# Jiang-Muyun/PointNet12

Measured on AMD Instinct MI355X. Metric: points/sec fwd+bwd, PointNet2 SemSeg B=16x4096 pts, higher is better.
Workload: dtype f32 (wide-layer products: exact bf16x3 operand splits, 6 bf16 MFMAs per fp32 product, fp32 accumulate)

## Files before the change

### pointnet12_amd/csrc/mlp_res.hip

```cpp
#include "mlp_loaders.h"
#include "split_bf16.h"
#include <algorithm>

int pn2_wide_fwd(const float *X, int ldx, const float *in_affine, const float *W, int ldw, const float *bias, float *Y, int ldy,
                 int64_t P, int K, int N, double *stats, LazyBn lz, hipStream_t s, int64_t *rows_done, int Kpool,
                 const float *pool_gamma, float *pool_ws);

namespace {

constexpr int RES_BM = 64;

struct ResPlan {
    signed char dx_rb[8], dx_cj[8];
    signed char dw_cj[8], dw_q0[8], dw_q1[8];
};

inline bool make_res_plan(int CI_T, ResPlan *out) {
    ResPlan p;
    int load[8], next_q[4] = {0, 0, 0, 0};
    for (int w = 0; w < 8; ++w) { p.dx_rb[w] = p.dx_cj[w] = -1; p.dw_cj[w] = 0; p.dw_q0[w] = p.dw_q1[w] = 0; load[w] = 0; }
    if (CI_T < 1 || CI_T > 4) return false;
    for (int i = 0; i < 2 * CI_T; ++i) { p.dx_rb[i] = (signed char)(i & 1); p.dx_cj[i] = (signed char)(i >> 1); load[i] = 2; }
    const int target = CI_T > 2 ? CI_T : 2;
    for (int pass = 0; pass < 2; ++pass)
// ... 686 lines not shown
                        const float4 a0 = xr[0], a1 = xr[1], a2 = xr[2];
                        g0[0] = __builtin_fmaf(dz, a0.x, g0[0]); g0[FUSE0 ? 1 : 0] = __builtin_fmaf(dz, a0.y, g0[FUSE0 ? 1 : 0]);
                        g0[FUSE0 ? 2 : 0] = __builtin_fmaf(dz, a0.z, g0[FUSE0 ? 2 : 0]); g0[FUSE0 ? 3 : 0] = __builtin_fmaf(dz, a0.w, g0[FUSE0 ? 3 : 0]);
                        g0[FUSE0 ? 4 : 0] = __builtin_fmaf(dz, a1.x, g0[FUSE0 ? 4 : 0]); g0[FUSE0 ? 5 : 0] = __builtin_fmaf(dz, a1.y, g0[FUSE0 ? 5 : 0]);
                        g0[FUSE0 ? 6 : 0] = __builtin_fmaf(dz, a1.z, g0[FUSE0 ? 6 : 0]); g0[FUSE0 ? 7 : 0] = __builtin_fmaf(dz, a1.w, g0[FUSE0 ? 7 : 0]);
                        g0[FUSE0 ? 8 : 0] = __builtin_fmaf(dz, a2.x, g0[FUSE0 ? 8 : 0]); g0[FUSE0 ? 9 : 0] = __builtin_fmaf(dz, a2.y, g0[FUSE0 ? 9 : 0]);
                        g0[FUSE0 ? 10 : 0] = __builtin_fmaf(dz, a2.z, g0[FUSE0 ? 10 : 0]); g0[FUSE0 ? 11 : 0] = __builtin_fmaf(dz, a2.w, g0[FUSE0 ? 11 : 0]);
                    } else {
#if defined(PN2_EXP_NOSTORE)
                        if (dz == 1.2345e-33f) xb[offx] = dz;
#elif defined(PN2_EXP_PLAINSTORE)
                        xb[offx] = dz;
#else
                        PN2_STREAM_STORE(dz, xb + offx);
#endif
                    }
                    offx += ((r & 3) == 3 ? 5u : 1u) * (unsigned)ldxo;
                }
                if (MASKED) { st0 += (double)s0; st1 += (double)s1; }
                RSTAMP(4)
            }
            chunk += G;
            buf ^= 1;
        };
        while (chunk < chunks) {
            iter(D2 ? raw1 : raw0);
            if (chunk >= chunks) break;
            iter(raw0);
        }
        RSTAMP_FLUSH(wave)
        RABS(wave, 2)
        if (!DXW) {
#pragma unroll
            for (int j = 0; j < TW; ++j) {
                const int e = (wave - CI_T) + j * NDW;
                if (e < NTILE) {
                    const int mb = e / CI_T, nb = e - mb * CI_T;
#pragma unroll
                    for (int r = 0; r < 16; ++r)
                        atomicAdd(dW + (int64_t)(mb * 32 + acc_row(r, lh)) * lddw + nb * 32 + l31, accw[DXW ? 0 : j][r]);
                }
            }
        } else if (MASKED && red_p != nullptr) {
            st0 += __shfl_xor(st0, 32, 64);
            st1 += __shfl_xor(st1, 32, 64);
            if (lh == 0) {
                double *rep = red_p + (size_t)(blockIdx.x % PN2_STAT_REPLICAS) * 2 * Ci;
                atomicAdd(rep + ecol, st0);
                atomicAdd(rep + Ci + ecol, st1);
            }
        }
        if (DXW && FUSE0) {
#pragma unroll
            for (int j = 0; j < (DXW && FUSE0 ? 12 : 1); ++j) g0[j] += __shfl_xor(g0[j], 32, 64);
            if (lh == 0) {
                float *pr = part0 + ((size_t)(blockIdx.x % PN2_CF_REPL) * Ci + ecol) * 16;
#pragma unroll
                for (int j = 0; j < (DXW && FUSE0 ? 12 : 1); ++j) atomicAdd(pr + j, g0[j]);
            }
        }
    };
    if (has_dx) run(pn2_true{}); else run(pn2_false{});
    RABS(wave, 3)
}

template <int CO_T, int CI_T, bool POOLED, bool MASKED, bool FUSE0 = false>
int launch_split_bwd_res(ResDy dy, const float *Yp, int ldp, const float *aff_p, const float *W, int ldw, int64_t tiles, float *dX, int ldxo,
                         double *red_p, float *dW, int lddw, hipStream_t s, const float *X0 = nullptr, int ld0 = 0, float *part0 = nullptr) {
    constexpr int Co = 32 * CO_T, Ci = 32 * CI_T;
    constexpr size_t lds = 2 * 6 * (size_t)(32 * 256) + sizeof(float) * (2 * 32 * (Ci + 4) + 8 * Co + 6 * Ci + (FUSE0 ? 2 * 32 * 12 : 0)) +
                           (CO_T == 4 && CI_T < 4 ? (size_t)CI_T * (Co / 16) * 1024 : 0);
    static_assert(lds <= 160 * 1024, "LDS");
    if ((reinterpret_cast<uintptr_t>(dy.Y) & 15) != 0 || (reinterpret_cast<uintptr_t>(Yp) & 15) != 0) return PN2_EUNSUPPORTED;
    auto kern = split_bwd_res_kernel<CO_T, CI_T, POOLED, MASKED, FUSE0>;
    static Pn2PerDevice raised;
    if (pn2_raise_dynamic_lds(reinterpret_cast<const void *>(kern), raised) != PN2_OK) return PN2_ELAUNCH;
    const int64_t chunks = tiles * (RES_BM / 32), cap = pn2_num_cus();
    PN2_NOTE_KERNEL(kern);
    hipLaunchKernelGGL(kern, dim3((unsigned)(chunks < cap ? chunks : cap)), dim3(512), lds, s, dy, Yp, ldp, aff_p, W, ldw, chunks, dX, ldxo,
                       red_p, dW, lddw, X0, ld0, part0);
    return pn2_launch_status();
}

template <int CO_T, int CI_T>
__global__ __launch_bounds__(512, 1) void split_bwd_cf_kernel(const float *dZp, const int32_t *arg, int ldo, int kshift, const float *W2 ,
                                                              const float *Yp, int ldp, const float *aff_p, int64_t chunks, float *dX, int ldxo, double *red_p,
                                                              float *slab) {
    constexpr int Co = 32 * CO_T, Ci = 32 * CI_T, BP = 32, QD = Co / 4, QP = Ci / 4, LDP = Ci + 4;
    constexpr int PANEL = BP * 256, BUF = 6 * PANEL;
    constexpr int KBX = Co / 16, KBM = Ci / 16, KBT = KBX + KBM;
    constexpr int NS = 8 - CI_T - 1, NTS = 64 * NS;
    constexpr int NGT = CI_T * (CI_T + 1) / 2, LDT = Co + Ci + 4;
    static_assert(NS >= CO_T, "one staging wave per D column");
    constexpr int RPP = NTS / QD, IT_D = (BP + RPP - 1) / RPP, IT_P = (BP * QP + NTS - 1) / NTS;
    static_assert(NTS % QD == 0, "one channel quad of D per staging thread");
    unsigned char *lds_b = reinterpret_cast<unsigned char *>(res_lds);
    float *Yps = res_lds + (2 * BUF) / 4;
    float *xtab = Yps + 2 * BP * LDP;
    const int t = threadIdx.x, lane = t & 63, wave = __builtin_amdgcn_readfirstlane(t >> 6), l31 = lane & 31, lh = lane >> 5;
    const int G = gridDim.x;
    RABS(wave, 0)
    for (int i = t; i < 3 * Ci; i += 512) { const float v = aff_p[i]; xtab[i] = v; xtab[3 * Ci + i] = i < Ci ? v : -v; }

    const bool has_dx = wave < CI_T, is_gram = wave == CI_T;
    const int ecol = (has_dx ? wave : 0) * 32 + l31;
    const int ts = wave <= CI_T ? 0 : t - 64 * (CI_T + 1);
    struct Raw { float4 z; int4 a; float4 p[IT_P]; };
    Raw raw;
    auto p_item = [&](int i, int &row, int &q) { const int idx = (NTS * (i + 1) > BP * QP) ? min(ts + NTS * i, BP * QP - 1) : ts + NTS * i; row = idx / QP; q = idx - row * QP; };
    auto fetch = [&](int64_t chunk) {
        const unsigned m0 = (unsigned)(chunk < chunks ? chunk : chunks - 1) * BP;
        const unsigned o = (m0 >> kshift) * (unsigned)ldo + 4u * (unsigned)(ts % QD);
        raw.z = ld4(dZp + o);
        raw.a = ld4i(arg + o);
#pragma unroll
        for (int i = 0; i < IT_P; ++i) {
            int row, q;
            p_item(i, row, q);
            raw.p[i] = ld4(Yp + ((m0 + (unsigned)row) * (unsigned)ldp + 4u * (unsigned)q));
        }
    };
    auto store_split = [&](unsigned char *img, int row, int q, const float4 v) {
        unsigned h0, m0, l0, h1, m1, l1;
        split2(v.x, v.y, h0, m0, l0);
        split2(v.z, v.w, h1, m1, l1);
        const unsigned o = tr_img_off(row, q >> 1) + 8u * (unsigned)(q & 1);
        *reinterpret_cast<uint2 *>(img + o) = make_uint2(h0, h1);
        *reinterpret_cast<uint2 *>(img + o + PANEL) = make_uint2(m0, m1);
        *reinterpret_cast<uint2 *>(img + o + 2 * PANEL) = make_uint2(l0, l1);
    };
    auto stage = [&](int64_t chunk, int buf) {
        unsigned char *ia = lds_b + buf * BUF, *ib = ia + 3 * PANEL;
        float *yp = Yps + buf * (BP * LDP);
        const unsigned m0 = (unsigned)(chunk < chunks ? chunk : chunks - 1) * BP;
        const int kbase = (int)(m0 & ((1u << kshift) - 1u));
        const int par = (int)(chunk & 1);
        const float *xt = xtab + par * (3 * Ci);
        const float lim = par ? -INFINITY : INFINITY;
        {
            unsigned h0, m0_, l0, h1, m1, l1;
            split2(raw.z.x, raw.z.y, h0, m0_, l0);
            split2(raw.z.z, raw.z.w, h1, m1, l1);
            const unsigned sm2 = par ? 0x80008000u : 0u;
            h0 ^= sm2; m0_ ^= sm2; l0 ^= sm2; h1 ^= sm2; m1 ^= sm2; l1 ^= sm2;
            const int q = ts % QD, r0 = ts / QD;
            const int4 a = raw.a;
#pragma unroll
            for (int i = 0; i < IT_D; ++i) {
                const int row = (RPP * (i + 1) > BP) ? min(r0 + RPP * i, BP - 1) : r0 + RPP * i;
                const int k = kbase + row;
                const unsigned k0 = (a.x == k ? 0x0000ffffu : 0u) | (a.y == k ? 0xffff0000u : 0u);
                const unsigned k1 = (a.z == k ? 0x0000ffffu : 0u) | (a.w == k ? 0xffff0000u : 0u);
                const unsigned o = tr_img_off(row, q >> 1) + 8u * (unsigned)(q & 1);
                *reinterpret_cast<uint2 *>(ia + o) = make_uint2(h0 & k0, h1 & k1);
                *reinterpret_cast<uint2 *>(ia + o + PANEL) = make_uint2(m0_ & k0, m1 & k1);
                *reinterpret_cast<uint2 *>(ia + o + 2 * PANEL) = make_uint2(l0 & k0, l1 & k1);
            }
        }
#pragma unroll
        for (int i = 0; i < IT_P; ++i) {
            int row, q;
            p_item(i, row, q);
            float4 x = raw.p[i];
            *reinterpret_cast<float4 *>(&yp[row * LDP + 4 * q]) = x;
            const float4 mu = *reinterpret_cast<const float4 *>(&xt[4 * q]), sc = *reinterpret_cast<const float4 *>(&xt[Ci + 4 * q]);
            const float4 be = *reinterpret_cast<const float4 *>(&xt[2 * Ci + 4 * q]);
            x.x = __builtin_amdgcn_fmed3f(bn_act(x.x, mu.x, sc.x, be.x), 0.f, lim); x.y = __builtin_amdgcn_fmed3f(bn_act(x.y, mu.y, sc.y, be.y), 0.f, lim);
            x.z = __builtin_amdgcn_fmed3f(bn_act(x.z, mu.z, sc.z, be.z), 0.f, lim); x.w = __builtin_amdgcn_fmed3f(bn_act(x.w, mu.w, sc.w, be.w), 0.f, lim);
            store_split(ib, row, q, x);
        }
    };
    auto raw_landed = [&]() {
        asm volatile("" : "+v"(raw.z.x), "+v"(raw.z.y), "+v"(raw.z.z), "+v"(raw.z.w));
        asm volatile("" : "+v"(raw.a.x), "+v"(raw.a.y), "+v"(raw.a.z), "+v"(raw.a.w));
#pragma unroll
        for (int i = 0; i < IT_P; ++i) asm volatile("" : "+v"(raw.p[i].x), "+v"(raw.p[i].y), "+v"(raw.p[i].z), "+v"(raw.p[i].w));
    };
    const int g16 = lane >> 4, j16 = lane & 15, tq = j16 >> 2, tp = j16 & 3;
    auto frag_t = [&](const unsigned char *img, int cblk, int pb) {
        const int c0 = (cblk * 32 + 16 * (g16 & 1)) >> 3;
        SplitFrag f;
#pragma unroll
        for (int r2 = 0; r2 < 2; ++r2) {
            const int row = 16 * pb + 8 * (g16 >> 1) + 4 * r2 + tq;
            const unsigned o = tr_img_off(row, c0 + (tp >> 1)) + 8u * (unsigned)(tp & 1);
            const pn2_s16x4 v = __builtin_amdgcn_ds_read_tr16_b64_v4i16(
                reinterpret_cast<__attribute__((address_space(3))) pn2_s16x4 *>((__attribute__((address_space(3))) unsigned char *)(img) + o));
            const uint2 u = __builtin_bit_cast(uint2, v);
            f.u[2 * r2] = u.x; f.u[2 * r2 + 1] = u.y;
        }
        return f;
    };

    if (has_dx) {
        SplitFrag wh[KBT], wm[KBT], wl[KBM];
        uint4 *wl_lds = reinterpret_cast<uint4 *>(xtab + 6 * Ci) + (size_t)wave * KBX * 64 + lane;
        {
            float v[KBT][8];
#pragma unroll
            for (int kb = 0; kb < KBT; ++kb)
#pragma unroll
                for (int e = 0; e < 8; ++e) v[kb][e] = W2[(16 * kb + 8 * lh + e) * Ci + ecol];
#pragma unroll
            for (int kb = 0; kb < KBT; ++kb) {
                SplitFrag lo;
#pragma unroll
                for (int e = 0; e < 4; ++e) split2(v[kb][2 * e], v[kb][2 * e + 1], wh[kb].u[e], wm[kb].u[e], lo.u[e]);
                if (kb < KBX) wl_lds[kb * 64] = lo.q; else wl[kb < KBX ? 0 : kb - KBX] = lo;
            }
        }
        Affine a(aff_p, Ci);
        const float emu = a.mean[ecol], esc = a.scale[ecol], ebe = a.beta[ecol], eis = a.invstd[ecol];
        const float eh = W2[(Co + Ci) * Ci + ecol];
        double st0 = 0.0, st1 = 0.0, st2 = 0.0;
        int64_t chunk = blockIdx.x;
        int buf = 0;
        __syncthreads();
        RABS(wave, 1)
        RSTAMP_DECL
        while (chunk < chunks) {
            __syncthreads();
            RSTAMP(2)
            const unsigned char *ia = lds_b + buf * BUF, *ib = ia + 3 * PANEL;
            f32x16 acc, acc2;
#pragma unroll
            for (int r = 0; r < 16; ++r) { acc[r] = 0.f; acc2[r] = 0.f; }
#ifndef PN2_X_CF_NODXM
#pragma unroll
            for (int kb = 0; kb < KBT; ++kb) {
                const unsigned char *img = kb < KBX ? ia : ib;
                const unsigned o = tr_img_off(l31, 2 * (kb < KBX ? kb : kb - KBX) + lh);
                SplitFrag ah, am, al, wlo;
                ah.q = *reinterpret_cast<const uint4 *>(img + o);
                am.q = *reinterpret_cast<const uint4 *>(img + o + PANEL);
                al.q = *reinterpret_cast<const uint4 *>(img + o + 2 * PANEL);
                if (kb < KBX) wlo.q = wl_lds[kb * 64]; else wlo = wl[kb < KBX ? 0 : kb - KBX];
                acc = __builtin_amdgcn_mfma_f32_32x32x16_bf16(al.v, wh[kb].v, acc, 0, 0, 0);
                acc2 = __builtin_amdgcn_mfma_f32_32x32x16_bf16(ah.v, wlo.v, acc2, 0, 0, 0);
                acc = __builtin_amdgcn_mfma_f32_32x32x16_bf16(am.v, wm[kb].v, acc, 0, 0, 0);
                acc2 = __builtin_amdgcn_mfma_f32_32x32x16_bf16(am.v, wh[kb].v, acc2, 0, 0, 0);
                acc = __builtin_amdgcn_mfma_f32_32x32x16_bf16(ah.v, wm[kb].v, acc, 0, 0, 0);
                acc2 = __builtin_amdgcn_mfma_f32_32x32x16_bf16(ah.v, wh[kb].v, acc2, 0, 0, 0);
            }
#endif
#ifdef PN2_STAMP
            { float a0_ = acc[0] + acc2[0]; asm volatile("" : "+v"(a0_)); }
#endif
            RSTAMP(3)
#ifdef PN2_X_CF_NOEPI
            if (acc[0] == 1.2345e-33f) dX[0] = acc2[1];
            chunk += G; buf ^= 1;
            continue;
#endif
            const float *yq = Yps + buf * (BP * LDP) + (4 * lh) * LDP + ecol;
            float yv[16];
#pragma unroll
            for (int r = 0; r < 16; ++r) yv[r] = yq[((r & 3) + 8 * (r >> 2)) * LDP];
// ... 27 lines not shown
        if (lh == 0) {
            if (red_p != nullptr) {
                double *rep = red_p + (size_t)(blockIdx.x % PN2_STAT_REPLICAS) * 2 * Ci;
                atomicAdd(rep + ecol, st0);
                atomicAdd(rep + Ci + ecol, st1);
            }
            slab[(size_t)blockIdx.x * (Ci * LDT) + (size_t)ecol * LDT + Co + Ci] = (float)st2;
        }
    } else {
        constexpr int PA[6] = {2, 0, 1, 1, 0, 0}, PB[6] = {0, 2, 1, 0, 1, 0};
        auto mm2 = [&](f32x16 &c0, const SplitFrag (&a0)[3], const SplitFrag (&b0)[3], f32x16 &c1, const SplitFrag (&a1)[3], const SplitFrag (&b1)[3]) {
#pragma unroll
            for (int q = 0; q < 6; ++q) {
                c0 = __builtin_amdgcn_mfma_f32_32x32x16_bf16(a0[PA[q]].v, b0[PB[q]].v, c0, 0, 0, 0);
                c1 = __builtin_amdgcn_mfma_f32_32x32x16_bf16(a1[PA[q]].v, b1[PB[q]].v, c1, 0, 0, 0);
            }
        };
        auto mm1 = [&](f32x16 &c0, const SplitFrag (&a0)[3], const SplitFrag (&b0)[3]) {
#pragma unroll
            for (int q = 0; q < 6; ++q) c0 = __builtin_amdgcn_mfma_f32_32x32x16_bf16(a0[PA[q]].v, b0[PB[q]].v, c0, 0, 0, 0);
        };
        auto frag3 = [&](const unsigned char *img, int blk, int pb, SplitFrag (&f)[3]) {
            f[0] = frag_t(img, blk, pb); f[1] = frag_t(img + PANEL, blk, pb); f[2] = frag_t(img + 2 * PANEL, blk, pb);
        };
        float *sl = slab + (size_t)blockIdx.x * (Ci * LDT);
        if (is_gram) {
            f32x16 accg[NGT];
#pragma unroll
            for (int j = 0; j < NGT; ++j)
#pragma unroll
                for (int r = 0; r < 16; ++r) accg[j][r] = 0.f;
            int64_t chunk = blockIdx.x;
            int buf = 0;
            __syncthreads();
            RABS(wave, 1)
            RSTAMP_DECL
            while (chunk < chunks) {
                __syncthreads();
                RSTAMP(2)
#ifndef PN2_X_CF_NOT
                const unsigned char *ib = lds_b + buf * BUF + 3 * PANEL;
#pragma unroll
                for (int pb = 0; pb < BP / 16; ++pb) {
                    SplitFrag fx[CI_T][3];
#pragma unroll
                    for (int i = 0; i < CI_T; ++i) frag3(ib, i, pb, fx[i]);
                    if constexpr (CI_T == 1) {
                        mm1(accg[0], fx[0], fx[0]);
                    } else if constexpr (CI_T == 2) {
                        mm2(accg[0], fx[0], fx[0], accg[1], fx[0], fx[1]);
                        mm1(accg[2], fx[1], fx[1]);
                    } else {
                        static_assert(CI_T <= 3, "Gram tiles");
                        mm2(accg[0], fx[0], fx[0], accg[1], fx[0], fx[1]);
                        mm2(accg[2], fx[1], fx[1], accg[3], fx[0], fx[2]);
                        mm2(accg[4], fx[1], fx[2], accg[5], fx[2], fx[2]);
                    }
                }
#endif
                RSTAMP(3)
                chunk += G;
                buf ^= 1;
            }
            RSTAMP_FLUSH(wave)
            RABS(wave, 2)
#pragma unroll
            for (int j = 0; j < CI_T; ++j)
#pragma unroll
                for (int i = 0; i <= j; ++i) {
                    const f32x16 &acc = accg[j * (j + 1) / 2 + i];
#pragma unroll
                    for (int r = 0; r < 16; ++r) sl[(i * 32 + acc_row(r, lh)) * LDT + Co + j * 32 + l31] = acc[r];
                    if (i != j) {
#pragma unroll
                        for (int r = 0; r < 16; ++r) sl[(j * 32 + l31) * LDT + Co + i * 32 + acc_row(r, lh)] = acc[r];
                    }
                }
        } else {
            f32x16 accw[CI_T];
#pragma unroll
            for (int j = 0; j < CI_T; ++j)
#pragma unroll
                for (int r = 0; r < 16; ++r) accw[j][r] = 0.f;
            const int nb = wave - CI_T - 1 < CO_T ? wave - CI_T - 1 : -1;
            int64_t chunk = blockIdx.x;
            fetch(chunk);
            __syncthreads();
            stage(chunk, 0);
            fetch(chunk + G);
            raw_landed();
            int buf = 0;
            RABS(wave, 1)
            RSTAMP_DECL
            while (chunk < chunks) {
                __syncthreads();
                RSTAMP(2)
#ifndef PN2_X_CF_NOSTAGE
                stage(chunk + G, buf ^ 1);
#endif
                RSTAMP(0)
#ifndef PN2_X_CF_NOFETCH
                fetch(chunk + 2 * (int64_t)G);
#endif
                __builtin_amdgcn_sched_barrier(0);
                RSTAMP(1)
#ifndef PN2_X_CF_NOT
                if (nb >= 0) {
                    const unsigned char *ia = lds_b + buf * BUF, *ib = ia + 3 * PANEL;
#pragma unroll
                    for (int pb = 0; pb < BP / 16; ++pb) {
                        SplitFrag fb[3], fa0[3], fa1[3];
                        frag3(ia, nb, pb, fb);
                        frag3(ib, 0, pb, fa0);
                        if constexpr (CI_T >= 2) {
                            frag3(ib, 1, pb, fa1);
                            mm2(accw[0], fa0, fb, accw[CI_T >= 2 ? 1 : 0], fa1, fb);
                            if constexpr (CI_T == 3) {
                                frag3(ib, 2, pb, fa0);
                                mm1(accw[CI_T == 3 ? 2 : 0], fa0, fb);
                            }
                        } else {
                            mm1(accw[0], fa0, fb);
                        }
                    }
                }
#endif
                RSTAMP(3)
                chunk += G;
                buf ^= 1;
            }
            RSTAMP_FLUSH(wave)
            RABS(wave, 2)
            if (nb >= 0) {
#pragma unroll
                for (int i = 0; i < CI_T; ++i)
#pragma unroll
                    for (int r = 0; r < 16; ++r) sl[(i * 32 + acc_row(r, lh)) * LDT + nb * 32 + l31] = accw[i][r];
            }
        }
    }
    RABS(wave, 3)
}

__global__ __launch_bounds__(128) void cf_prep_kernel(LazyCoef lc, const float *coef, int ldc, const float *__restrict__ W, int ldw,
                                                      const float *__restrict__ bias, int Co, int Ci, float *__restrict__ W2) {
    __shared__ double fac[256];
    lazy_coef_prologue(lc);
    const float *c0 = coef, *q1 = coef + ldc, *q0 = coef + 2 * ldc, *mean = coef + 3 * ldc;
    const int r = blockIdx.x;
    if (r < Co) {
        for (int i = threadIdx.x; i < Ci; i += 128) W2[r * Ci + i] = c0[r] * W[(int64_t)r * ldw + i];
        return;
    }
    const int j = r - Co;
    for (int c = threadIdx.x; c < Co; c += 128)
        fac[c] = j == Ci ? ((double)q1[c] * ((double)bias[c] - (double)mean[c]) + (double)q0[c]) : (double)W[(int64_t)c * ldw + j] * (double)q1[c];
    __syncthreads();
    for (int i = threadIdx.x; i < Ci; i += 128) {
        double s0 = 0.0, s1 = 0.0, s2 = 0.0, s3 = 0.0;
#pragma unroll 4
        for (int c = 0; c < Co; c += 4) {
            s0 += fac[c] * (double)W[(int64_t)c * ldw + i];
            s1 += fac[c + 1] * (double)W[(int64_t)(c + 1) * ldw + i];
            s2 += fac[c + 2] * (double)W[(int64_t)(c + 2) * ldw + i];
            s3 += fac[c + 3] * (double)W[(int64_t)(c + 3) * ldw + i];
        }
        W2[r * Ci + i] = (float)((s0 + s1) + (s2 + s3));
    }
}

__global__ __launch_bounds__(256) void cf_finish_kernel(const float *__restrict__ slab, int nslab, int Co, int Ci, const float *coef, int ldc,
                                                        const float *__restrict__ W, int ldw, const float *__restrict__ bias,
                                                        float *__restrict__ dW, int lddw) {
    extern __shared__ double cf_row[];
    const int i = blockIdx.x, LDT = Co + Ci + 4, NQ = LDT / 4;
    const int q = threadIdx.x & 63, sg = threadIdx.x >> 6;
    double a0 = 0.0, a1 = 0.0, a2 = 0.0, a3 = 0.0;
    if (q < NQ) {
        const float *p = slab + (size_t)i * LDT + 4 * q;
        const size_t ss = (size_t)Ci * LDT;
        int w = sg;
        for (; w + 28 < nslab; w += 32) {
            float4 v[8];
#pragma unroll
            for (int e = 0; e < 8; ++e) v[e] = ld4(p + (size_t)(w + 4 * e) * ss);
#pragma unroll
            for (int e = 0; e < 8; ++e) { a0 += (double)v[e].x; a1 += (double)v[e].y; a2 += (double)v[e].z; a3 += (double)v[e].w; }
        }
        for (; w < nslab; w += 4) {
            const float4 v = ld4(p + (size_t)w * ss);
            a0 += (double)v.x; a1 += (double)v.y; a2 += (double)v.z; a3 += (double)v.w;
        }
        double *d = cf_row + sg * LDT + 4 * q;
        d[0] = a0; d[1] = a1; d[2] = a2; d[3] = a3;
    }
    __syncthreads();
    for (int n = threadIdx.x; n < LDT; n += 256) cf_row[n] = (cf_row[n] + cf_row[LDT + n]) + (cf_row[2 * LDT + n] + cf_row[3 * LDT + n]);
    __syncthreads();
    const float *c0 = coef, *q1 = coef + ldc, *q0 = coef + 2 * ldc, *mean = coef + 3 * ldc;
    const double sx = cf_row[Co + Ci];
    for (int c = threadIdx.x; c < Co; c += 256) {
        double dot = 0.0;
        for (int j = 0; j < Ci; ++j) dot += (double)W[(int64_t)c * ldw + j] * cf_row[Co + j];
        const double g = (double)c0[c] * cf_row[c] + (double)q1[c] * (dot + ((double)bias[c] - (double)mean[c]) * sx) + (double)q0[c] * sx;
        dW[(int64_t)c * lddw + i] += (float)g;
    }
}

template <int CO_T, int CI_T>
int launch_split_bwd_cf(const float *dZp, const int32_t *arg, int ldo, int kshift, const float *coef, LazyCoef lc, const float *W, int ldw,
                        const float *bias, const float *Yp, int ldp, const float *aff_p, int64_t P, float *dX, int ldxo, double *red_p,
                        float *dW, int lddw, float *scratch, hipStream_t s) {
    constexpr int Co = 32 * CO_T, Ci = 32 * CI_T, LDT = Co + Ci + 4;
    constexpr size_t lds = 2 * 6 * (size_t)(32 * 256) + sizeof(float) * (2 * 32 * (Ci + 4) + 6 * Ci) + (size_t)CI_T * (Co / 16) * 1024;
    static_assert(lds <= 160 * 1024, "LDS");
    auto kern = split_bwd_cf_kernel<CO_T, CI_T>;
    static Pn2PerDevice raised;
    if (pn2_raise_dynamic_lds(reinterpret_cast<const void *>(kern), raised) != PN2_OK) return PN2_ELAUNCH;
    float *W2 = scratch, *slab = scratch + (((Co + Ci + 1) * Ci + 63) & ~63);
    const int64_t chunks = P / 32, cap = pn2_num_cus() < 256 ? pn2_num_cus() : 256;
    const int grid = (int)(chunks < cap ? chunks : cap);
    hipLaunchKernelGGL(cf_prep_kernel, dim3(Co + Ci + 1), dim3(128), 0, s, lc, coef, (Co + 3) & ~3, W, ldw, bias, Co, Ci, W2);
    PN2_NOTE_KERNEL(kern);
    hipLaunchKernelGGL(kern, dim3((unsigned)grid), dim3(512), lds, s, dZp, arg, ldo, kshift, W2, Yp, ldp, aff_p, chunks, dX, ldxo, red_p, slab);
    hipLaunchKernelGGL(cf_finish_kernel, dim3(Ci), dim3(256), sizeof(double) * 4 * LDT, s, slab, grid, Co, Ci, coef, (Co + 3) & ~3, W, ldw, bias,
                       dW, lddw);
    return pn2_launch_status();
}

#define PN2_RES_CASE(CO, CI, POOL, MASKED)                                                                                \
    if (Co == CO && Ci == CI)                                                                                              \
        return launch_bwd_res<CO / 32, CI / 32, POOL, MASKED>(dy, Yp, ldp, aff_p, W, ldw, tiles, dX, ldxo, red_p, dW, lddw, s);

int dispatch_bwd_res(int Kpool, bool masked, int Co, int Ci, ResDy dy, const float *Yp, int ldp, const float *aff_p, const float *W,
                     int ldw, int64_t tiles, float *dX, int ldxo, double *red_p, float *dW, int lddw, hipStream_t s) {
    if (pn2_opt(PN2_OPT_SPLIT) && pn2_opt(PN2_OPT_SPLIT_RES)) {
#define PN2_SPLIT_RES_CASE(CO, CI, POOLED, MASKED)                                                                        \
        if (Co == CO && Ci == CI) {                                                                                        \
            const int rc = launch_split_bwd_res<CO / 32, CI / 32, POOLED, MASKED>(dy, Yp, ldp, aff_p, W, ldw, tiles, dX, ldxo, red_p, dW, lddw, s); \
            if (rc != PN2_EUNSUPPORTED) return rc;                                                                         \
        }
        const bool all = pn2_opt(PN2_OPT_SPLIT_RES) >= 2;
        if (Kpool == 0 && masked) {
            if (all) { PN2_SPLIT_RES_CASE(32, 32, false, true) }
            PN2_SPLIT_RES_CASE(64, 64, false, true) PN2_SPLIT_RES_CASE(96, 64, false, true)
            if (tiles >= pn2_opt(PN2_OPT_SPLIT_RES_MIN_TILES_128)) { PN2_SPLIT_RES_CASE(128, 128, false, true) }
        } else if (Kpool == 0) {
            if (tiles >= pn2_opt(PN2_OPT_SPLIT_RES_MIN_TILES_128)) { PN2_SPLIT_RES_CASE(128, 128, false, false) }
        } else if (masked && Kpool % 32 == 0) {
            if (all) { PN2_SPLIT_RES_CASE(64, 32, true, true) }
            PN2_SPLIT_RES_CASE(128, 64, true, true) PN2_SPLIT_RES_CASE(128, 96, true, true)
        }
#undef PN2_SPLIT_RES_CASE
    }
    if (Kpool == 0 && masked) {
        PN2_RES_CASE(32, 32, 0, true) PN2_RES_CASE(64, 64, 0, true) PN2_RES_CASE(96, 64, 0, true)
        if (tiles >= 4096) { PN2_RES_CASE(128, 128, 0, true) }
    } else if (Kpool == 0) {
        if (tiles >= 4096) { PN2_RES_CASE(128, 128, 0, false) }
    } else if (masked && Kpool % 64 == 0) {
        PN2_RES_CASE(128, 64, 1, true) PN2_RES_CASE(128, 96, 1, true)
    } else if (masked && Kpool == 32) {
        PN2_RES_CASE(64, 32, 2, true) PN2_RES_CASE(128, 64, 2, true)
    }
    return PN2_EUNSUPPORTED;
}

struct ResPool {
    float2 *rec;
    const float *gamma;
    int ldp, U;
    LazyBn lz;
};

template <int K_T, int N_T, bool ACT, int POOL>
__global__ __launch_bounds__(512, 2) void fwd_res_kernel(const float *__restrict__ X, int ldx, const float *aff ,
                                                         const float *__restrict__ W, int ldw, const float *__restrict__ bias,
                                                         float *__restrict__ Y, int ldy, int64_t slabs, double *__restrict__ stats,
                                                         ResPool pool) {
    constexpr int K = 32 * K_T, N = 32 * N_T, LDA = K + 4, QK = K / 4, IT = 32 * QK / 64;
    const int NW = blockDim.x >> 6;
    float *Ws = res_lds;
    float *atab = Ws + N * LDA;
    const int t = threadIdx.x, lane = t & 63, wave = __builtin_amdgcn_readfirstlane(t >> 6), l31 = lane & 31, lh = lane >> 5;
    float *Ab = atab + 3 * K + wave * (32 * LDA);
    RABS(wave, 0)

    lazy_bn_prologue(pool.lz);
    for (int i = t; i < N * QK; i += blockDim.x) {
        const int n = i / QK, q = i - n * QK;
        const float *src = W + (int64_t)n * ldw + 4 * q;
        float4 v;
        if ((ldw & 3) == 0 && (reinterpret_cast<uintptr_t>(W) & 15) == 0) v = ld4(src);
        else v = make_float4(src[0], src[1], src[2], src[3]);
        *reinterpret_cast<float4 *>(&Ws[n * LDA + 4 * q]) = v;
    }
    if (ACT)
        for (int i = t; i < 3 * K; i += blockDim.x) atab[i] = aff[i];
    float bj[N_T];
// ... 326 lines not shown

extern "C" int pn2_bn_pool_select(const float *pool_ws, const float *affine, int64_t G, int C, float *out, int ldo, int32_t *arg,
                                  const pn2_bn_lazy *lazy, pn2_stream_t stream) {
    PN2_CHECK_ARG(lazy_bn_ok(lazy, affine, C));
    PN2_CHECK_ARG(pool_ws && affine && out && arg && G > 0 && C > 0 && C % 32 == 0 && ldo >= C && ldo % 4 == 0 &&
                  (reinterpret_cast<uintptr_t>(pool_ws) & 15) == 0 && (reinterpret_cast<uintptr_t>(out) & 15) == 0);
    const int64_t n = G * (C >> 2);
    int64_t blocks = pn2_cdiv(n, 256);
    const int64_t cap = (int64_t)pn2_num_cus() * 8;
    if (blocks > cap) blocks = cap;
    hipLaunchKernelGGL(bn_pool_select_kernel, dim3((unsigned)blocks), dim3(256), 0, pn2_s(stream),
                       reinterpret_cast<const float2 *>(pool_ws), C, affine, C, G, C, out, ldo, arg, make_lazy_bn(lazy));
    return pn2_launch_status();
}

extern "C" int pn2_conv1x1_bwd(const float *dZ, int ldz, const float *dZp, int ldo, const int32_t *arg, int Kpool, const float *Y,
                               int ldy, const float *coef, const float *W, int ldw, const float *prev_Y, int ld_prev,
                               const float *prev_affine, float *dXout, int ldxo, double *prev_red, float *dW, int lddw,
                               int64_t P, int C_out, int C_in, const pn2_bn_coef_lazy *coef_lazy, pn2_stream_t stream) {
    PN2_CHECK_ARG(Y && coef && W && prev_Y && dXout && dW && P > 0 && P < (1LL << 31) && res_shape_ok(C_out, C_in));
    PN2_CHECK_ARG(lazy_coef_ok(coef_lazy, coef, C_out));
    PN2_CHECK_ARG(dZ != nullptr || (dZp && arg && Kpool > 0));
    PN2_CHECK_ARG(ldw >= C_in && lddw >= C_in && ldy % 4 == 0 && ldy >= C_out && ld_prev % 4 == 0 && ld_prev >= C_in && ldxo >= C_in);
    PN2_CHECK_ARG(prev_affine != nullptr || prev_red == nullptr);
    hipStream_t s = pn2_s(stream);
    const int kshift = dZ ? 0 : pow2_shift(Kpool);
    PN2_CHECK_ARG(dZ ? (ldz == ldy) : (kshift >= 0 && ldo % 4 == 0 && ldo >= C_out && prev_affine != nullptr && P % Kpool == 0));
    int64_t tiles = P / RES_BM, P_full = tiles * RES_BM;
    int rc = PN2_OK;
    const int64_t ld_max = std::max(std::max((int64_t)ldy, (int64_t)ld_prev), std::max((int64_t)ldxo, dZ ? (int64_t)ldz : (int64_t)ldo));
    if (P * ld_max >= (1LL << 32)) { tiles = 0; P_full = 0; }
    if (tiles > 0) {
        ResDy dy{dZ, dZp, arg, ldo, kshift, Y, ldy, coef, make_lazy_coef(coef_lazy)};
        rc = dispatch_bwd_res(dZ ? 0 : Kpool, prev_affine != nullptr, C_out, C_in, dy, prev_Y, ld_prev, prev_affine, W, ldw, tiles, dXout, ldxo,
                              prev_red, dW, lddw, s);
        if (rc == PN2_EUNSUPPORTED) { rc = PN2_OK; tiles = 0; P_full = 0; }
        else coef_lazy = nullptr;
    }
    if (rc != PN2_OK || P_full == P) return rc;
    const int64_t tail = P - P_full;
    const int64_t g_off = dZ ? 0 : (P_full / Kpool) * ldo;
    const float *dZt = dZ ? dZ + P_full * ldz : nullptr;
    const float *dZpt = dZ ? nullptr : dZp + g_off;
    const int32_t *argt = dZ ? nullptr : arg + g_off;
    rc = pn2_conv1x1_dgrad(dZt, ldz, dZpt, ldo, argt, Kpool, Y + P_full * ldy, ldy, coef, W, ldw, prev_affine ? prev_Y + P_full * ld_prev : nullptr,
                           ld_prev, prev_affine, dXout + P_full * ldxo, ldxo, prev_red, tail, C_out, C_in, coef_lazy, stream);
    if (rc != PN2_OK) return rc;
    return pn2_conv1x1_wgrad(dZt, ldz, dZpt, ldo, argt, Kpool, Y + P_full * ldy, ldy, coef, prev_Y + P_full * ld_prev, ld_prev, prev_affine,
                             dW, lddw, nullptr, tail, C_out, C_in, nullptr, stream);
}

static bool cf_shape(int C_out, int C_in) { return C_out == 128 && (C_in == 96 || C_in == 64); }

extern "C" int pn2_conv1x1_bwd_cf_supported(int64_t P, int C_out, int C_in, int Kpool) {
    if (!(pn2_opt(PN2_OPT_SPLIT) && pn2_opt(PN2_OPT_SPLIT_RES) && pn2_opt(PN2_OPT_POOL_CF))) return 0;
    if (!pn2_res_supported(P, C_out, C_in) || !cf_shape(C_out, C_in)) return 0;
    if (C_in == 64 && pn2_opt(PN2_OPT_POOL_CF) < 2) return 0;
    if (Kpool < 32 || (Kpool & (Kpool - 1)) != 0 || P % Kpool != 0) return 0;
    if (P * (int64_t)std::max(C_out, C_in) >= (1LL << 32)) return 0;
    return 1;
}

extern "C" int64_t pn2_conv1x1_bwd_cf_scratch_bytes(int C_out, int C_in) {
    if (!cf_shape(C_out, C_in)) return 0;
    const int64_t w2 = (((int64_t)(C_out + C_in + 1) * C_in + 63) & ~63LL);
    return 4 * (w2 + 256LL * C_in * (C_out + C_in + 4));
}

extern "C" int pn2_conv1x1_bwd_cf(const float *dZp, int ldo, const int32_t *arg, int Kpool, const float *coef, const float *W, int ldw,
                                  const float *bias, const float *prev_Y, int ld_prev, const float *prev_affine, float *dXout, int ldxo,
                                  double *prev_red, float *dW, int lddw, int64_t P, int C_out, int C_in, const pn2_bn_coef_lazy *coef_lazy,
                                  float *scratch, pn2_stream_t stream) {
    PN2_CHECK_ARG(dZp && arg && coef && W && bias && prev_Y && prev_affine && dXout && dW && scratch && P > 0 && P < (1LL << 31));
    PN2_CHECK_ARG(lazy_coef_ok(coef_lazy, coef, C_out));
    PN2_CHECK_ARG(ldw >= C_in && lddw >= C_in && ld_prev % 4 == 0 && ld_prev >= C_in && ldxo >= C_in && ldo % 4 == 0 && ldo >= C_out);
    PN2_CHECK_ARG((reinterpret_cast<uintptr_t>(scratch) & 255) == 0 && (reinterpret_cast<uintptr_t>(prev_Y) & 15) == 0 &&
                  (reinterpret_cast<uintptr_t>(dZp) & 15) == 0 && (reinterpret_cast<uintptr_t>(arg) & 15) == 0);
    if (!pn2_conv1x1_bwd_cf_supported(P, C_out, C_in, Kpool)) return PN2_EUNSUPPORTED;
    const int64_t ld_max = std::max(std::max((int64_t)ld_prev, (int64_t)ldxo), (int64_t)ldo);
    if (P * ld_max >= (1LL << 32)) return PN2_EUNSUPPORTED;
    const int kshift = pow2_shift(Kpool);
    const LazyCoef lc = make_lazy_coef(coef_lazy);
    hipStream_t s = pn2_s(stream);
    if (C_in == 96) return launch_split_bwd_cf<4, 3>(dZp, arg, ldo, kshift, coef, lc, W, ldw, bias, prev_Y, ld_prev, prev_affine, P, dXout, ldxo, prev_red, dW, lddw, scratch, s);
    return launch_split_bwd_cf<4, 2>(dZp, arg, ldo, kshift, coef, lc, W, ldw, bias, prev_Y, ld_prev, prev_affine, P, dXout, ldxo, prev_red, dW, lddw, scratch, s);
}

extern "C" int pn2_conv1x1_bwd_first_supported(int64_t P, int C_out, int C_in, int N0) {
    if (!(pn2_opt(PN2_OPT_SPLIT) && pn2_opt(PN2_OPT_SPLIT_RES) && pn2_opt(PN2_OPT_FUSE_FIRST))) return 0;
    if (!pn2_res_supported(P, C_out, C_in) || P % 64 != 0 || N0 < 1 || N0 > 12) return 0;
    if (P * (int64_t)std::max(C_out, C_in) >= (1LL << 32)) return 0;
    return (C_out == 96 && C_in == 64) || (C_out == 64 && C_in == 64);
}

extern "C" int pn2_conv1x1_bwd_first(const float *dZ, int ldz, const float *Y, int ldy, const float *coef, const float *W, int ldw,
                                     const float *prev_Y, int ld_prev, const float *prev_affine, double *prev_red, float *dW, int lddw,
                                     const float *X0, int ld0, int N0, void *cf_scratch, int64_t P, int C_out, int C_in,
                                     const pn2_bn_coef_lazy *coef_lazy, pn2_stream_t stream) {
    PN2_CHECK_ARG(dZ && Y && coef && W && prev_Y && prev_affine && prev_red && dW && X0 && cf_scratch && P > 0 && P < (1LL << 31));
    PN2_CHECK_ARG(lazy_coef_ok(coef_lazy, coef, C_out));
    PN2_CHECK_ARG(ldz == ldy && ldw >= C_in && lddw >= C_in && ldy % 4 == 0 && ldy >= C_out && ld_prev % 4 == 0 && ld_prev >= C_in);
    PN2_CHECK_ARG(ld0 % 4 == 0 && ld0 >= 12 && (reinterpret_cast<uintptr_t>(X0) & 15) == 0 && (reinterpret_cast<uintptr_t>(cf_scratch) & 15) == 0);
    if (!pn2_conv1x1_bwd_first_supported(P, C_out, C_in, N0)) return PN2_EUNSUPPORTED;
    if (P * (int64_t)std::max((int64_t)ldy, std::max((int64_t)ld_prev, (int64_t)ld0)) >= (1LL << 32)) return PN2_EUNSUPPORTED;
    float *part0 = reinterpret_cast<float *>(reinterpret_cast<double *>(cf_scratch) + PN2_CF_REPL * 256);
    ResDy dy{dZ, nullptr, nullptr, 0, 0, Y, ldy, coef, make_lazy_coef(coef_lazy)};
    const int64_t tiles = P / RES_BM;
    hipStream_t s = pn2_s(stream);
    if (C_out == 96) return launch_split_bwd_res<3, 2, false, true, true>(dy, prev_Y, ld_prev, prev_affine, W, ldw, tiles, nullptr, 0, prev_red, dW, lddw, s, X0, ld0, part0);
    return launch_split_bwd_res<2, 2, false, true, true>(dy, prev_Y, ld_prev, prev_affine, W, ldw, tiles, nullptr, 0, prev_red, dW, lddw, s, X0, ld0, part0);
}
```

### pointnet12_amd/csrc/pn2_common.h

```cpp
#pragma once
#include <hip/hip_runtime.h>
#include <stdint.h>
#include <mutex>
#include <set>
#include <utility>
#include "../../include/pn2.h"

#define PN2_WAVE 64
#define PN2_CF_REPL 8

#ifdef PN2_PLAIN_STORES
#define PN2_STREAM_STORE(value, ptr) (*(ptr) = (value))
#else
#define PN2_STREAM_STORE(value, ptr) __builtin_nontemporal_store((value), (ptr))
#endif

#define PN2_CHECK_ARG(cond) \
    do {                    \
        if (!(cond)) return PN2_EINVAL; \
    } while (0)

static inline int pn2_launch_status() { return hipGetLastError() == hipSuccess ? PN2_OK : PN2_ELAUNCH; }

static inline hipStream_t pn2_s(pn2_stream_t s) { return reinterpret_cast<hipStream_t>(s); }

static inline int64_t pn2_cdiv(int64_t a, int64_t b) { return (a + b - 1) / b; }

#define PN2_OPTION_LIST(X) \
    X(FPS_ROWS_MIN_PPT, 24)  \
    X(FPS_ROWMAP, 2)  \
    X(FPS_SINGLE_MAX, 24576)  \
    X(FPS_PIECE, 0)  \
    X(FPS_COOP, 1)  \
    X(FPS_PRUNE, 1)  \
    X(BQ_ORDER, 1)  \
    X(FEWROW_MAX_TILES, 1024)  \
    X(FEWROW_MAX_TILES_DGRAD, 512)  \
    X(FEWROW_KS, 0)  \
    X(NT_CFG, 0)  \
    X(NT_SMALL_DEPTH, 1)  \
    X(NT_NSPLIT, 1)  \
    X(TN_SPLITDIV, 1)  \
    X(TN_CFG, 0)  \
    X(TN_NARROW, 1)  \
    X(TN_SMALLP, 65536)  \
    X(TN_SMALL_DEPTH, 2)  \
    X(CF_WGS_PER_CU, 2)  \
    X(WGRAD_SKINNY, 1)  \
    X(BWD_PAIR, 1)  \
    X(RES, 1)  \
    X(RES_MIN_ROWS, 32768)  \
    X(RES_HALF, 1)  \
    X(WIDE, 1)  \
    X(WIDE_MIN_ROWS, 65536)  \
    X(SPLIT, 1)  \
    X(SPLIT_WGRAD, 1)  \
    X(SPLIT_K256, 1)  \
    X(SPLIT_NARROW, 1)  \
    X(SPLIT_RES, 1)  \
    X(FUSE_FIRST, 1)  \
    X(SPLIT_WG2, 1)  \
    X(POOL_CF, 2)  \
    X(SPLIT_RES_MIN_TILES_128, 1024)  \
    X(SPLIT_MIN_ROWS_128, 98304)  \
    X(RING, 0)  \
    X(WIDE_POOL, 1)  \
    X(WIDE_ADB196, 1)  \
    X(WIDE_WGRAD, 1)  \
    X(WIDE_WGRAD_MIN_ROWS, 131072)  \
    X(WGRAD_TWO_PHASE, 0)  \
    X(WGRAD_TWO_PHASE_ALL, 0)  \
    X(SEG_CHUNK, 0)

enum Pn2Option {
#define PN2_X(name, dflt) PN2_OPT_##name,
    PN2_OPTION_LIST(PN2_X)
#undef PN2_X
    PN2_OPT_COUNT
};
extern int pn2_option_table[PN2_OPT_COUNT];
static inline int pn2_opt(int id) { return __atomic_load_n(&pn2_option_table[id], __ATOMIC_RELAXED); }

extern thread_local const void *pn2_last_kernel_fn;
#define PN2_NOTE_KERNEL(...) (pn2_last_kernel_fn = reinterpret_cast<const void *>(__VA_ARGS__))

#define PN2_MAX_DEVICES 16
static inline int pn2_device_slot() {
    int dev = 0;
    if (hipGetDevice(&dev) != hipSuccess || dev < 0) dev = 0;
    return dev < PN2_MAX_DEVICES ? dev : PN2_MAX_DEVICES - 1;
}

static inline int pn2_num_cus() {
    static int cus[PN2_MAX_DEVICES] = {0};
    const int slot = pn2_device_slot();
    if (cus[slot] == 0) {
        int dev = 0;
        hipDeviceProp_t prop;
        int n = 0;
        if (hipGetDevice(&dev) == hipSuccess && hipGetDeviceProperties(&prop, dev) == hipSuccess) n = prop.multiProcessorCount;
        cus[slot] = n > 0 ? n : 256;
    }
    return cus[slot];
}

struct Pn2PerDevice {
    bool flag[PN2_MAX_DEVICES] = {false};
    bool get() const { return flag[pn2_device_slot()]; }
    void set() { flag[pn2_device_slot()] = true; }
};
static inline int pn2_raise_dynamic_lds(const void *kernel, Pn2PerDevice &done) {
    if (done.get()) return PN2_OK;
    if (hipFuncSetAttribute(kernel, hipFuncAttributeMaxDynamicSharedMemorySize, 160 * 1024) != hipSuccess) return PN2_ELAUNCH;
    done.set();
    return PN2_OK;
}

static inline int pn2_raise_dynamic_lds_once(const void *kernel) {
    static std::mutex mu;
    static std::set<std::pair<const void *, int>> done;
    const std::pair<const void *, int> key(kernel, pn2_device_slot());
    std::lock_guard<std::mutex> lock(mu);
    if (done.count(key)) return PN2_OK;
    if (hipFuncSetAttribute(kernel, hipFuncAttributeMaxDynamicSharedMemorySize, 160 * 1024) != hipSuccess) return PN2_ELAUNCH;
    done.insert(key);
    return PN2_OK;
}

#define PN2_OPAQUE1(a) asm volatile("" : "+v"(a))
#define PN2_OPAQUE3(a, b, c) asm volatile("" : "+v"(a), "+v"(b), "+v"(c))
#define PN2_OPAQUE4(a, b, c, d) asm volatile("" : "+v"(a), "+v"(b), "+v"(c), "+v"(d))

__device__ __forceinline__ unsigned long long pn2_wave_max_u64(unsigned long long v) {
#pragma unroll
    for (int m = 32; m >= 1; m >>= 1) {
        unsigned long long o = __shfl_xor(v, m, 64);
        v = o > v ? o : v;
    }
    return v;
}

__device__ __forceinline__ unsigned pn2_row_max_u32(unsigned v) {
    asm volatile("s_nop 1\n\t"
                 "v_max_u32_dpp %0, %0, %0 quad_perm:[1,0,3,2] row_mask:0xf bank_mask:0xf\n\t"
                 "s_nop 1\n\t"
// ... 71 lines not shown
```

Before: 13.13 million.

## Use one-hot MFMA for pooled gradient in CF backward weight-gradient path

New measurement: 13.29 million, median of 5. About the same (+1.2%).

```diff
diff --git a/pointnet12_amd/csrc/mlp_res.hip b/pointnet12_amd/csrc/mlp_res.hip
--- a/pointnet12_amd/csrc/mlp_res.hip
+++ b/pointnet12_amd/csrc/mlp_res.hip
@@ -792,7 +792,7 @@
     return pn2_launch_status();
 }
 
-template <int CO_T, int CI_T>
+template <int CO_T, int CI_T, bool ONEHOT>
 __global__ __launch_bounds__(512, 1) void split_bwd_cf_kernel(const float *dZp, const int32_t *arg, int ldo, int kshift, const float *W2 ,
                                                               const float *Yp, int ldp, const float *aff_p, int64_t chunks, float *dX, int ldxo, double *red_p,
                                                               float *slab) {
@@ -815,7 +815,9 @@
     const bool has_dx = wave < CI_T, is_gram = wave == CI_T;
     const int ecol = (has_dx ? wave : 0) * 32 + l31;
     const int ts = wave <= CI_T ? 0 : t - 64 * (CI_T + 1);
-    struct Raw { float4 z; int4 a; float4 p[IT_P]; };
+    const int nb = wave > CI_T && wave - CI_T - 1 < CO_T ? wave - CI_T - 1 : -1;
+    const unsigned vcol = 32u * (unsigned)(nb < 0 ? 0 : nb) + (unsigned)l31;
+    struct Raw { float4 z; int4 a; float4 p[IT_P]; float v; int av; };
     Raw raw;
     auto p_item = [&](int i, int &row, int &q) { const int idx = (NTS * (i + 1) > BP * QP) ? min(ts + NTS * i, BP * QP - 1) : ts + NTS * i; row = idx / QP; q = idx - row * QP; };
     auto fetch = [&](int64_t chunk) {
@@ -823,6 +825,11 @@
         const unsigned o = (m0 >> kshift) * (unsigned)ldo + 4u * (unsigned)(ts % QD);
         raw.z = ld4(dZp + o);
         raw.a = ld4i(arg + o);
+        if constexpr (ONEHOT) {
+            const unsigned ov = (m0 >> kshift) * (unsigned)ldo + vcol;
+            raw.v = dZp[ov];
+            raw.av = arg[ov];
+        }
 #pragma unroll
         for (int i = 0; i < IT_P; ++i) {
             int row, q;
@@ -883,6 +890,7 @@
     auto raw_landed = [&]() {
         asm volatile("" : "+v"(raw.z.x), "+v"(raw.z.y), "+v"(raw.z.z), "+v"(raw.z.w));
         asm volatile("" : "+v"(raw.a.x), "+v"(raw.a.y), "+v"(raw.a.z), "+v"(raw.a.w));
+        if constexpr (ONEHOT) asm volatile("" : "+v"(raw.v), "+v"(raw.av));
 #pragma unroll
         for (int i = 0; i < IT_P; ++i) asm volatile("" : "+v"(raw.p[i].x), "+v"(raw.p[i].y), "+v"(raw.p[i].z), "+v"(raw.p[i].w));
     };
@@ -1076,11 +1084,12 @@
             for (int j = 0; j < CI_T; ++j)
 #pragma unroll
                 for (int r = 0; r < 16; ++r) accw[j][r] = 0.f;
-            const int nb = wave - CI_T - 1 < CO_T ? wave - CI_T - 1 : -1;
             int64_t chunk = blockIdx.x;
             fetch(chunk);
             __syncthreads();
             stage(chunk, 0);
+            float v0 = ONEHOT ? raw.v : 0.f, v1 = 0.f;
+            int a0 = ONEHOT ? raw.av : 0, a1 = 0;
             fetch(chunk + G);
             raw_landed();
             int buf = 0;
@@ -1092,6 +1101,7 @@
 #ifndef PN2_X_CF_NOSTAGE
                 stage(chunk + G, buf ^ 1);
 #endif
+                if constexpr (ONEHOT) { v1 = raw.v; a1 = raw.av; }
                 RSTAMP(0)
 #ifndef PN2_X_CF_NOFETCH
                 fetch(chunk + 2 * (int64_t)G);
@@ -1099,7 +1109,32 @@
                 __builtin_amdgcn_sched_barrier(0);
                 RSTAMP(1)
 #ifndef PN2_X_CF_NOT
-                if (nb >= 0) {
+                if (ONEHOT && nb >= 0) {
+                    const unsigned char *ib = lds_b + buf * BUF + 3 * PANEL;
+                    const int d0 = a0 - (int)(((unsigned)chunk * BP) & ((1u << kshift) - 1u)) - 8 * lh;
+                    const unsigned one = (chunk & 1) ? 0xbf80u : 0x3f80u;
+                    f32x16 pc[CI_T];
+#pragma unroll
+                    for (int i = 0; i < CI_T; ++i)
+#pragma unroll
+                        for (int r = 0; r < 16; ++r) pc[i][r] = 0.f;
+#pragma unroll
+                    for (int pb = 0; pb < BP / 16; ++pb) {
+                        SplitFrag fe, fx[CI_T][3];
+#pragma unroll
+                        for (int j = 0; j < 4; ++j) fe.u[j] = (d0 - 16 * pb == 2 * j ? one : 0u) | (d0 - 16 * pb == 2 * j + 1 ? one << 16 : 0u);
+#pragma unroll
+                        for (int i = 0; i < CI_T; ++i) frag3(ib, i, pb, fx[i]);
+#pragma unroll
+                        for (int q = 2; q >= 0; --q)
+#pragma unroll
+                            for (int i = 0; i < CI_T; ++i) pc[i] = __builtin_amdgcn_mfma_f32_32x32x16_bf16(fx[i][q].v, fe.v, pc[i], 0, 0, 0);
+                    }
+#pragma unroll
+                    for (int i = 0; i < CI_T; ++i)
+#pragma unroll
+                        for (int r = 0; r < 16; ++r) accw[i][r] = __builtin_fmaf(v0, pc[i][r], accw[i][r]);
+                } else if (nb >= 0) {
                     const unsigned char *ia = lds_b + buf * BUF, *ib = ia + 3 * PANEL;
 #pragma unroll
                     for (int pb = 0; pb < BP / 16; ++pb) {
@@ -1120,6 +1155,7 @@
                 }
 #endif
                 RSTAMP(3)
+                v0 = v1; a0 = a1;
                 chunk += G;
                 buf ^= 1;
             }
@@ -1201,14 +1237,14 @@
     }
 }
 
-template <int CO_T, int CI_T>
+template <int CO_T, int CI_T, bool ONEHOT>
 int launch_split_bwd_cf(const float *dZp, const int32_t *arg, int ldo, int kshift, const float *coef, LazyCoef lc, const float *W, int ldw,
                         const float *bias, const float *Yp, int ldp, const float *aff_p, int64_t P, float *dX, int ldxo, double *red_p,
                         float *dW, int lddw, float *scratch, hipStream_t s) {
     constexpr int Co = 32 * CO_T, Ci = 32 * CI_T, LDT = Co + Ci + 4;
     constexpr size_t lds = 2 * 6 * (size_t)(32 * 256) + sizeof(float) * (2 * 32 * (Ci + 4) + 6 * Ci) + (size_t)CI_T * (Co / 16) * 1024;
     static_assert(lds <= 160 * 1024, "LDS");
-    auto kern = split_bwd_cf_kernel<CO_T, CI_T>;
+    auto kern = split_bwd_cf_kernel<CO_T, CI_T, ONEHOT>;
     static Pn2PerDevice raised;
     if (pn2_raise_dynamic_lds(reinterpret_cast<const void *>(kern), raised) != PN2_OK) return PN2_ELAUNCH;
     float *W2 = scratch, *slab = scratch + (((Co + Ci + 1) * Ci + 63) & ~63);
@@ -1701,8 +1737,10 @@
     const int kshift = pow2_shift(Kpool);
     const LazyCoef lc = make_lazy_coef(coef_lazy);
     hipStream_t s = pn2_s(stream);
-    if (C_in == 96) return launch_split_bwd_cf<4, 3>(dZp, arg, ldo, kshift, coef, lc, W, ldw, bias, prev_Y, ld_prev, prev_affine, P, dXout, ldxo, prev_red, dW, lddw, scratch, s);
-    return launch_split_bwd_cf<4, 2>(dZp, arg, ldo, kshift, coef, lc, W, ldw, bias, prev_Y, ld_prev, prev_affine, P, dXout, ldxo, prev_red, dW, lddw, scratch, s);
+#define PN2_CF_ARGS dZp, arg, ldo, kshift, coef, lc, W, ldw, bias, prev_Y, ld_prev, prev_affine, P, dXout, ldxo, prev_red, dW, lddw, scratch, s
+    if (pn2_opt(PN2_OPT_CF_ONEHOT)) return C_in == 96 ? launch_split_bwd_cf<4, 3, true>(PN2_CF_ARGS) : launch_split_bwd_cf<4, 2, true>(PN2_CF_ARGS);
+    return C_in == 96 ? launch_split_bwd_cf<4, 3, false>(PN2_CF_ARGS) : launch_split_bwd_cf<4, 2, false>(PN2_CF_ARGS);
+#undef PN2_CF_ARGS
 }
 
 extern "C" int pn2_conv1x1_bwd_first_supported(int64_t P, int C_out, int C_in, int N0) {
diff --git a/pointnet12_amd/csrc/pn2_common.h b/pointnet12_amd/csrc/pn2_common.h
--- a/pointnet12_amd/csrc/pn2_common.h
+++ b/pointnet12_amd/csrc/pn2_common.h
@@ -61,6 +61,7 @@
     X(FUSE_FIRST, 1)  \
     X(SPLIT_WG2, 1)  \
     X(POOL_CF, 2)  \
+    X(CF_ONEHOT, 1)  \
     X(SPLIT_RES_MIN_TILES_128, 1024)  \
     X(SPLIT_MIN_ROWS_128, 98304)  \
     X(RING, 0)  \
```
